# willi-menapace/PlayableEnvironments

Measured on AMD Instinct MI355X. Metric: Mrays/s, higher is better.
Workload: dtype f32; 1 GPU; tennis renderer, 256x256 frame per GPU (rank r renders the frame of seed 1234 + r), 4 objects, 64+128 hierarchical samples/ray (coarse+fine networks), eval - BASELINE.json configs[1]; rays_per_gpu=65536, frames_per_gpu=1, parallelism=frame shard x1

## Files before the change

### playableenvironments_amd/csrc/composite.hip

```cpp
#include "pr_common.h"
#include "composite_dev.h"

namespace pr {

struct CompositeSmem {
    float* tt;
    float* sg;
    float* dm;
    float* wo;
    float* wg;
    float* al;
    float* dv;
    int* sl;
    unsigned int* key;
};

constexpr int MAX_FCHUNK = 4;

__device__ __forceinline__ void transmittance_weights(float* al, int n, int lane) {
    float carry = 1.0f;
    for (int base = 0; base < n; base += 64) {
        const int j = base + lane;
        const float a = (j < n) ? al[j] : 0.f;
        float incl = (j < n) ? __fadd_rn(__fsub_rn(1.0f, a), 1e-10f) : 1.0f;
// ... 28 lines not shown
        const float a = (j < end) ? al[j] : 0.f;
        float incl = (j < end) ? __fadd_rn(__fsub_rn(1.0f, a), 1e-10f) : 1.0f;
#pragma unroll
        for (int d = 1; d < 64; d <<= 1) {
            const float o = __shfl_up(incl, d, 64);
            if (lane >= d) incl *= o;
        }
        float excl = __shfl_up(incl, 1, 64);
        if (lane == 0) excl = 1.0f;
        if (j < end) al[j] = a * (carry * excl);
        carry *= __shfl(incl, 63, 64);
    }
    if (lane == 0) totals[wave] = carry;
    __syncthreads();
    float before = 1.0f;
    for (int w = 0; w < wave; ++w) before *= totals[w];
    if (wave > 0)
        for (int j = begin + lane; j < end; j += 64) al[j] *= before;
    __syncthreads();
}

template <int CW>
__device__ __forceinline__ float block_sum(float v, float* scratch, int wave, int lane) {
    v = wave_sum(v);
    if (CW == 1) return v;
    __syncthreads();
    if (lane == 0) scratch[wave] = v;
    __syncthreads();
    float total = 0.f;
    for (int w = 0; w < CW; ++w) total += scratch[w];
    return total;
}

template <int CW>
__device__ __forceinline__ void store_channel_sums(float (&acc)[MAX_FCHUNK], float* dst, int F, float* scratch, int wave, int lane) {
    if (CW > 1) {
#pragma unroll
        for (int c = 0; c < MAX_FCHUNK; ++c) {
            if (64 * c >= F) break;
            __syncthreads();
            scratch[wave * 64 + lane] = acc[c];
            __syncthreads();
            if (wave == 0)
                for (int w = 1; w < CW; ++w) acc[c] = __fadd_rn(acc[c], scratch[w * 64 + lane]);
        }
    }
    if (wave == 0) {
#pragma unroll
        for (int c = 0; c < MAX_FCHUNK; ++c) {
            const int ch = lane + 64 * c;
            if (ch < F) dst[ch] = acc[c];
        }
    }
}

template <int CW>
__global__ __launch_bounds__(64 * CW) void k_composite(CompositeParams p) {
    extern __shared__ __attribute__((aligned(16))) char raw_smem[];
    constexpr int CT = 64 * CW;
    const int S = p.sort_size;
    CompositeSmem sm;
    const int A = (p.total_positions + 63) & ~63;
    sm.key = reinterpret_cast<unsigned int*>(raw_smem);
    sm.tt = reinterpret_cast<float*>(sm.key + S);
    sm.sg = sm.tt + A;
    sm.dm = sm.sg + A;
    sm.wo = sm.dm + A;
    sm.wg = sm.sg;
    sm.al = sm.wo + A;
    const bool use_div = p.any_divergence != 0;
    sm.dv = use_div ? sm.al + A : nullptr;
    sm.sl = reinterpret_cast<int*>(sm.al + (use_div ? 2 * A : A));
    float* scratch = reinterpret_cast<float*>(sm.sl + A);
    unsigned long long* wide = p.fix_overlaps ? reinterpret_cast<unsigned long long*>(scratch + 4 * 64) : nullptr;

    const int tid = threadIdx.x, lane = tid & 63;
    const int wave = (CW == 1) ? 0 : __builtin_amdgcn_readfirstlane(tid >> 6);
    const long g = blockIdx.x;
    const float* d = p.ray_directions + (size_t)g * 3;
    const float norm = sqrtf(__fadd_rn(__fadd_rn(__fmul_rn(d[0], d[0]), __fmul_rn(d[1], d[1])), __fmul_rn(d[2], d[2])));
    const int PT = p.total_positions;

    {
        int off = 0;
        for (int k = 0; k < p.objects; ++k) {
// ... 116 lines not shown
        sm.al[j] = alpha_of(raw, __fmul_rn(dt, norm));
        if (use_div) gdiv += sm.al[j] * sm.dv[e];
    }
    __syncthreads();
    transmittance_weights_block<CW>(sm.al, PT, scratch, wave, lane);
    if (CW == 1) __syncthreads();
    {
        float depth = 0.f, opacity = 0.f, dmag = 0.f;
        for (int j = tid; j < PT; j += CT) {
            const int e = (int)sm.key[j];
            const float w = sm.al[j];
            sm.wg[e] = w;
            if (p.global.weights) p.global.weights[gbase + j] = w;
            depth += w * sm.tt[e];
            opacity += w;
            dmag += w * sm.dm[e];
        }
        depth = block_sum<CW>(depth, scratch, wave, lane);
        opacity = block_sum<CW>(opacity, scratch, wave, lane);
        dmag = block_sum<CW>(dmag, scratch, wave, lane);
        if (use_div) gdiv = block_sum<CW>(gdiv, scratch, wave, lane);
        if (tid == 0) {
            if (p.global.depth) p.global.depth[g] = depth;
            if (p.global.opacity) p.global.opacity[g] = opacity;
            if (p.global.disparity) p.global.disparity[g] = disparity_of(depth, opacity);
            if (p.global.integrated_displacements_magnitude)
                p.global.integrated_displacements_magnitude[g] = dmag / (float)PT;
            if (p.global.integrated_divergence) p.global.integrated_divergence[g] = gdiv / (float)PT;
        }
    }
    __syncthreads();

    const int F = p.F;
    const bool defer = p.pooled != nullptr;
    int* lrow = reinterpret_cast<int*>(sm.key);
    float* lw1 = sm.tt;
    float accg[MAX_FCHUNK];
#pragma unroll
    for (int c = 0; c < MAX_FCHUNK; ++c) accg[c] = 0.f;
    int off = 0;
    for (int k = 0; k < p.objects; ++k) {
        const CompositeObject& o = p.obj[k];
        const int P = o.positions;
        const int part = (((P + CW - 1) / CW) + 63) & ~63;
        const int begin = wave * part;
        const int end = (begin + part < P) ? begin + part : P;
        __syncthreads();
        int count = 0;
        float bare1 = 0.f, bare2 = 0.f;
        for (int base = begin; base < end; base += 64) {
            const int i = base + lane;
            bool take = false;
            int row = -1;
            float w1 = 0.f, w2 = 0.f;
            if (i < end) {
                row = sm.sl[off + i];
                w1 = sm.wo[off + i];
                w2 = sm.wg[off + i];
                take = row >= 0 && (w1 != 0.f || w2 != 0.f);
                if (p.sigmoid && row < 0) {
                    bare1 += w1;
                    bare2 += w2;
                }
            }
            const unsigned long long m = __ballot(take);
            if (take) {
                const int pos = off + begin + count + __popcll(m & ((1ull << lane) - 1ull));
                lrow[pos] = row;
                lw1[pos] = w1;
                sm.al[pos] = w2;
            }
            count += __popcll(m);
        }
        const int* rows_w = lrow + off + begin;
        const float* w1_w = lw1 + off + begin;
        const float* w2_w = sm.al + off + begin;
        float acco[MAX_FCHUNK];
#pragma unroll
        for (int c = 0; c < MAX_FCHUNK; ++c) acco[c] = 0.f;
        int i = 0;
        for (; i + ROWS_IN_FLIGHT <= count; i += ROWS_IN_FLIGHT) {
            float v[ROWS_IN_FLIGHT][MAX_FCHUNK];
#pragma unroll
            for (int u = 0; u < ROWS_IN_FLIGHT; ++u) {
                const float* f = o.feat + (size_t)rows_w[i + u] * F;
#pragma unroll
                for (int c = 0; c < MAX_FCHUNK; ++c) {
                    const int ch = lane + 64 * c;
                    v[u][c] = (ch < F) ? f[ch] : 0.f;
                    if (p.sigmoid) v[u][c] = sigmoid_of(v[u][c]);
                }
            }
#pragma unroll
            for (int u = 0; u < ROWS_IN_FLIGHT; ++u) {
                const float w1 = w1_w[i + u], w2 = w2_w[i + u];
#pragma unroll
                for (int c = 0; c < MAX_FCHUNK; ++c) {
                    acco[c] = __fadd_rn(acco[c], __fmul_rn(w1, v[u][c]));
                    accg[c] = __fadd_rn(accg[c], __fmul_rn(w2, v[u][c]));
                }
            }
        }
        for (; i < count; ++i) {
            const float* f = o.feat + (size_t)rows_w[i] * F;
            const float w1 = w1_w[i], w2 = w2_w[i];
#pragma unroll
            for (int c = 0; c < MAX_FCHUNK; ++c) {
                const int ch = lane + 64 * c;
                float v = (ch < F) ? f[ch] : 0.f;
                if (p.sigmoid) v = sigmoid_of(v);
                acco[c] = __fadd_rn(acco[c], __fmul_rn(w1, v));
                accg[c] = __fadd_rn(accg[c], __fmul_rn(w2, v));
            }
        }
        if (p.sigmoid) {
            bare1 = wave_sum(bare1);
            bare2 = wave_sum(bare2);
#pragma unroll
            for (int c = 0; c < MAX_FCHUNK; ++c) {
                acco[c] = __fadd_rn(acco[c], 0.5f * bare1);
                accg[c] = __fadd_rn(accg[c], 0.5f * bare2);
            }
        }
        if (o.out.integrated_features)
            store_channel_sums<CW>(acco, defer ? p.pooled + ((size_t)(2 * k) * gridDim.x + g) * F : o.out.integrated_features + (size_t)g * F, F,
                                   scratch, wave, lane);
        if (defer) {
            if (p.global.integrated_features || p.decoder.groups > 0)
                store_channel_sums<CW>(accg, p.pooled + ((size_t)(2 * k + 1) * gridDim.x + g) * F, F, scratch, wave, lane);
#pragma unroll
            for (int c = 0; c < MAX_FCHUNK; ++c) accg[c] = 0.f;
        }
        off += P;
    }
    if (defer) return;
    if (p.global.integrated_features) store_channel_sums<CW>(accg, p.global.integrated_features + (size_t)g * F, F, scratch, wave, lane);
    if (p.decoder.groups > 0) {
        if (CW > 1 && !p.global.integrated_features) {
#pragma unroll
            for (int c = 0; c < MAX_FCHUNK; ++c) {
                if (64 * c >= F) break;
                __syncthreads();
                scratch[wave * 64 + lane] = accg[c];
                __syncthreads();
                if (wave == 0)
                    for (int w = 1; w < CW; ++w) accg[c] = __fadd_rn(accg[c], scratch[w * 64 + lane]);
            }
        }
        if (wave == 0) {
            const int frame = (int)(g / p.rays);
            int r = (int)(g - (long)frame * p.rays);
            int grp = 0;
            while (grp < p.decoder.groups - 1 && r >= p.decoder.rays[grp]) r -= p.decoder.rays[grp++];
            const int c0 = p.decoder.channel_begin[grp], c1 = p.decoder.channel_end[grp];
            const size_t cells = (size_t)p.decoder.rays[grp];
            float* map = p.decoder.map[grp] + (size_t)frame * (c1 - c0) * cells + r;
#pragma unroll
            for (int c = 0; c < MAX_FCHUNK; ++c) {
                const int ch = lane + 64 * c;
                if (ch >= c0 && ch < c1 && ch < F) map[(size_t)(ch - c0) * cells] = accg[c];
            }
        }
    }
}

int launch_composite(const CompositeParams& p, hipStream_t s) {
    PR_REQUIRE(p.F <= 64 * MAX_FCHUNK, "output_features %d exceeds %d", p.F, 64 * MAX_FCHUNK);
    PR_REQUIRE(p.sort_size >= p.total_positions && (p.sort_size & (p.sort_size - 1)) == 0, "bad sort size");
    for (int k = 0; k < p.objects; ++k)
        PR_REQUIRE(p.obj[k].positions <= 64 * 32, "positions per ray %d too large for the overlap mask", p.obj[k].positions);
    const size_t lds = (size_t)p.sort_size * 4 + (size_t)((p.total_positions + 63) & ~63) * (p.any_divergence ? 7 : 6) * 4 +
                       sizeof(float) * 4 * 64 + (p.fix_overlaps ? (size_t)p.sort_size * 8 : 0);
    PR_REQUIRE(lds <= 156 * 1024, "too many samples per ray for the compositing kernel (%d)", p.total_positions);
    if (p.decoder.groups > 0) {
        PR_REQUIRE(p.decoder.groups <= PR_MAX_DECODER_GROUPS, "decoder layout: %d groups (max %d)", p.decoder.groups, PR_MAX_DECODER_GROUPS);
        long sum = 0;
        for (int i = 0; i < p.decoder.groups; ++i) {
            PR_REQUIRE(p.decoder.rays[i] > 0 && p.decoder.width[i] > 0 && p.decoder.rays[i] % p.decoder.width[i] == 0,
                       "decoder layout: group %d has %d rays in rows of %d", i, p.decoder.rays[i], p.decoder.width[i]);
            PR_REQUIRE(p.decoder.channel_begin[i] >= 0 && p.decoder.channel_begin[i] < p.decoder.channel_end[i] && p.decoder.channel_end[i] <= (p.pooled ? p.out_features : p.F),
                       "decoder layout: group %d channel range [%d, %d) outside 0..%d", i, p.decoder.channel_begin[i], p.decoder.channel_end[i], p.pooled ? p.out_features : p.F);
            PR_REQUIRE(p.decoder.map[i] != nullptr, "decoder layout: group %d has no map", i);
            sum += p.decoder.rays[i];
        }
        PR_REQUIRE(sum == p.rays, "decoder layout: the groups hold %ld rays, the call has %d", sum, p.rays);
    }
    const long total = (long)p.frames * p.rays;
    ProfileScope scope(1, s);
    if (p.total_positions >= 256) {
        PR_TRY(prepare_kernel(reinterpret_cast<const void*>(&k_composite<4>), 156 * 1024, nullptr));
        hipLaunchKernelGGL(k_composite<4>, dim3((unsigned)total), dim3(256), lds, s, p);
    } else {
// ... 109 lines not shown
```

### playableenvironments_amd/csrc/geometry.hip

```cpp
#include "pr_common.h"

namespace pr {

__global__ void k_camera_rays(int frames, int rays, int per_frame, float half_h, float half_w, const float* __restrict__ c2w,
                              const float* __restrict__ focals, const int32_t* __restrict__ rows,
                              const int32_t* __restrict__ cols, float* __restrict__ origins,
                              float* __restrict__ dirs, float* __restrict__ normals) {
    const long g = (long)blockIdx.x * blockDim.x + threadIdx.x;
    const long total = (long)frames * rays;
    if (g >= total) return;
    const int n = (int)(g / rays);
    const int r = (int)(g - (long)n * rays);
    const float* m = c2w + (size_t)n * 12;
    const float f = focals[n];
    const long pix = per_frame ? g : (long)r;
    const float dx = __fdiv_rn(__fsub_rn((float)cols[pix], half_w), f);
    const float dy = -__fdiv_rn(__fsub_rn((float)rows[pix], half_h), f);
    const float dz = -1.0f;
#pragma unroll
    for (int i = 0; i < 3; ++i) {
        const float v = __fadd_rn(__fadd_rn(__fmul_rn(dx, m[i * 4 + 0]), __fmul_rn(dy, m[i * 4 + 1])),
                                  __fmul_rn(dz, m[i * 4 + 2]));
        dirs[g * 3 + i] = v;
    }
// ... 283 lines not shown
    PR_LAUNCH_CHECK();
    hipLaunchKernelGGL(k_fill_group, dim3(blocks, count), dim3(256), 0, s, fg);
    PR_LAUNCH_CHECK();
    return PR_OK;
}

int launch_fill(const FillParams& p, hipStream_t s) {
    const long total = (long)p.frames * p.rays;
    const int blocks = (int)((total + 255) / 256);
    hipLaunchKernelGGL(k_fill, dim3(blocks), dim3(256), 0, s, p);
    PR_LAUNCH_CHECK();
    return PR_OK;
}

__device__ __forceinline__ void bitonic_sort_f32(float* key, int n , int lane) {
    for (int k = 2; k <= n; k <<= 1) {
        for (int j = k >> 1; j > 0; j >>= 1) {
            for (int i = lane; i < n; i += 64) {
                const int x = i ^ j;
                if (x > i) {
                    const float a = key[i], b = key[x];
                    const bool up = ((i & k) == 0);
                    if ((a > b) == up) {
                        key[i] = b;
                        key[x] = a;
                    }
                }
            }
            __syncthreads();
        }
    }
}

__global__ __launch_bounds__(64) void k_resample(ResampleParams p, int sort_size) {
    extern __shared__ float sm[];
    if (p.skip && *p.skip) return;
    const int Pc = p.pc, Pf = p.pf;
    float* tc = sm;
    float* al = tc + Pc;
    float* mids = al + Pc;
    float* cdf = mids + Pc;
    float* key = cdf + Pc;
    const int lane = threadIdx.x;
    const long g = blockIdx.x;
    const int n = (int)(g / p.rays);
    const float* m = p.w2o + ((size_t)n * p.objects + p.object_index) * 12;
    const ObjRay ray = object_ray(m, p.ray_origins + (size_t)n * 3, p.ray_directions + (size_t)g * 3);
    const bool valid = p.in_scene[(size_t)n * p.objects + p.object_index] != 0;
    const float norm = sqrtf(__fadd_rn(__fadd_rn(__fmul_rn(ray.d[0], ray.d[0]), __fmul_rn(ray.d[1], ray.d[1])),
                                       __fmul_rn(ray.d[2], ray.d[2])));
    const size_t cbase = (size_t)g * Pc;
    for (int i = lane; i < Pc; i += 64) tc[i] = p.t_coarse[cbase + i];
    __syncthreads();
    for (int i = lane; i < Pc; i += 64) {
        float raw = valid ? p.sigma_coarse[cbase + i] : p.empty_alpha;
        if (noise_present(p.alpha_noise)) raw = __fadd_rn(raw, noise_normal(p.alpha_noise, g, Pc, i));
        const float dt = (i < Pc - 1) ? __fsub_rn(tc[i + 1], tc[i]) : 1e10f;
        const float dist = __fmul_rn(dt, norm);
        const float relu = raw > 0.f ? raw : 0.f;
        al[i] = __fsub_rn(1.0f, expf(__fmul_rn(-relu, dist)));
        if (i < Pc - 1) mids[i] = __fdiv_rn(__fadd_rn(tc[i + 1], tc[i]), 2.0f);
    }
    __syncthreads();
    if (lane == 0) {
        float trans = 1.0f;
        for (int i = 0; i < Pc; ++i) {
            const float a = al[i];
            al[i] = __fmul_rn(a, trans);
            trans = __fmul_rn(trans, __fadd_rn(__fsub_rn(1.0f, a), 1e-10f));
        }
        const int nb = Pc - 2;
        float sum = 0.f;
        for (int j = 0; j < nb; ++j) sum = __fadd_rn(sum, __fadd_rn(al[j + 1], 1e-5f));
        float c = 0.f;
        cdf[0] = 0.f;
        for (int j = 0; j < nb; ++j) {
            c = __fadd_rn(c, __fdiv_rn(__fadd_rn(al[j + 1], 1e-5f), sum));
            cdf[j + 1] = c;
        }
    }
    __syncthreads();
    const int ncdf = Pc - 1;
    for (int i = lane; i < sort_size; i += 64) key[i] = (i < Pc) ? tc[i] : __builtin_inff();
    for (int f = lane; f < Pf; f += 64) {
        const float u = noise_present(p.u_random) ? noise_uniform(p.u_random, g, Pf, f) : p.u_fixed[f];
        int lo_i = 0, hi_i = ncdf;
        while (lo_i < hi_i) {
            const int mid = (lo_i + hi_i) >> 1;
            if (cdf[mid] > u) hi_i = mid; else lo_i = mid + 1;
        }
        const int below = lo_i - 1 < 0 ? 0 : lo_i - 1;
        const int above = lo_i > ncdf - 1 ? ncdf - 1 : lo_i;
        float den = __fsub_rn(cdf[above], cdf[below]);
        if (den < 1e-5f) den = 1.0f;
        const float frac = __fdiv_rn(__fsub_rn(u, cdf[below]), den);
        key[Pc + f] = __fadd_rn(mids[below], __fmul_rn(frac, __fsub_rn(mids[above], mids[below])));
    }
    __syncthreads();
    const int Pm = Pc + Pf;
    float* merged = key + sort_size;
    bool sorted = true;
    for (int i = lane; i + 1 < Pc; i += 64) sorted = sorted && (key[i] <= key[i + 1]);
    for (int f = lane; f + 1 < Pf; f += 64) sorted = sorted && (key[Pc + f] <= key[Pc + f + 1]);
    if (__ballot(sorted) == ~0ull) {
        for (int i = lane; i < Pc; i += 64) {
            const float t = key[i];
            int lo = 0, hi = Pf;
            while (lo < hi) {
                const int mid = (lo + hi) >> 1;
                if (key[Pc + mid] < t) lo = mid + 1; else hi = mid;
            }
            merged[i + lo] = t;
        }
        for (int f = lane; f < Pf; f += 64) {
            const float t = key[Pc + f];
            int lo = 0, hi = Pc;
            while (lo < hi) {
                const int mid = (lo + hi) >> 1;
                if (key[mid] <= t) lo = mid + 1; else hi = mid;
            }
            merged[f + lo] = t;
        }
        __syncthreads();
    } else {
        bitonic_sort_f32(key, sort_size, lane);
        merged = key;
    }
    const size_t fbase = (size_t)g * Pm;
    int count = 0;
    for (int i = lane; i < Pm; i += 64) {
        const float t = merged[i];
        p.t_fine[fbase + i] = t;
        p.sigma_fine[fbase + i] = p.empty_alpha;
        if (p.dispmag_fine) p.dispmag_fine[fbase + i] = 0.f;
        const float x = __fadd_rn(ray.o[0], __fmul_rn(ray.d[0], t));
        const float y = __fadd_rn(ray.o[1], __fmul_rn(ray.d[1], t));
        const float z = __fadd_rn(ray.o[2], __fmul_rn(ray.d[2], t));
        if (sample_kept(x, y, z, p.lo, p.hi, p.occ, n)) ++count;
    }
#pragma unroll
    for (int d = 32; d > 0; d >>= 1) count += __shfl_down(count, d, 64);
    if (lane == 0 && count) atomicAdd(&p.block_sums[g >> 8], count);
}

__global__ __launch_bounds__(256) void k_expected_positions(int frames, int rays, int objects, int object_index, int P,
                                                            const float* ray_origins, const float* ray_directions,
                                                            const float* w2o, const float* t, const float* weights,
                                                            const float* delta, float* expected) {
    const long g = (long)blockIdx.x * 256 + threadIdx.x;
    if (g >= (long)frames * rays) return;
    const int n = (int)(g / rays);
    const ObjRay ray = object_ray(w2o + ((size_t)n * objects + object_index) * 12, ray_origins + (size_t)n * 3,
                                  ray_directions + (size_t)g * 3);
    const size_t base = (size_t)g * P;
    float acc[3] = {0.f, 0.f, 0.f}, wsum = 0.f;
    for (int i = 0; i < P; ++i) {
        const float ti = t[base + i], w = weights[base + i];
        for (int a = 0; a < 3; ++a) {
            float x = __fadd_rn(ray.o[a], __fmul_rn(ray.d[a], ti));
            if (delta) x = __fadd_rn(x, delta[(base + i) * 3 + a]);
            acc[a] = __fadd_rn(acc[a], __fmul_rn(x, w));
        }
        wsum = __fadd_rn(wsum, w);
    }
    for (int a = 0; a < 3; ++a) expected[(size_t)g * 3 + a] = __fdiv_rn(acc[a], __fadd_rn(wsum, 1e-8f));
}

static int next_pow2(int v) {
    int r = 1;
    while (r < v) r <<= 1;
    return r;
}

int launch_resample(const ResampleParams& p, hipStream_t s) {
    PR_REQUIRE(p.pc >= 3, "hierarchical sampling needs at least 3 coarse positions (got %d)", p.pc);
    const long total = (long)p.frames * p.rays;
    const int nblocks256 = (int)((total + 255) / 256);
    PR_TRY(launch_zero_fill(p.block_sums, sizeof(int32_t) * nblocks256, s));
    int sort_size = next_pow2(p.pc + p.pf);
    if (sort_size < 64) sort_size = 64;
    const size_t lds = sizeof(float) * (4 * (size_t)p.pc + 2 * (size_t)sort_size);
    PR_REQUIRE(lds <= 64 * 1024, "resample: too many positions per ray (%d + %d)", p.pc, p.pf);
    hipLaunchKernelGGL(k_resample, dim3((unsigned)total), dim3(64), lds, s, p, sort_size);
    PR_LAUNCH_CHECK();
    return PR_OK;
}

}

extern "C" int pr_expected_positions(int32_t frames, int32_t rays, int32_t objects, int32_t object_index, int32_t positions,
                                     const float* ray_origins, const float* ray_directions, const float* w2o, const float* t,
                                     const float* weights, const float* delta, float* expected, void* stream) {
    PR_REQUIRE(frames > 0 && rays > 0 && positions > 0 && objects > 0 && object_index >= 0 && object_index < objects,
               "pr_expected_positions: bad sizes");
    PR_REQUIRE(ray_origins && ray_directions && w2o && t && weights && expected, "pr_expected_positions: NULL pointer");
    const long total = (long)frames * rays;
    hipLaunchKernelGGL(pr::k_expected_positions, dim3((unsigned)((total + 255) / 256)), dim3(256), 0, (hipStream_t)stream, frames,
                       rays, objects, object_index, positions, ray_origins, ray_directions, w2o, t, weights, delta, expected);
    PR_LAUNCH_CHECK();
    return PR_OK;
}

namespace pr {
struct PatchPixelsParams {
    int frames, objects, height, width, patch, nstrides;
    int strides[4];
    const float* boxes;
    const float* weights;
    const float* u;
    int32_t* rows; int32_t* cols;
    int rays;
};

__global__ __launch_bounds__(256) void k_patch_pixels(PatchPixelsParams p) {
    __shared__ int start[2];
    const int n = blockIdx.x;
// ... 457 lines not shown
```

### playableenvironments_amd/csrc/pr_common.h

```cpp
#pragma once

#include <hip/hip_runtime.h>
#include <stdint.h>
#include <stdio.h>
#include <string.h>

#include "playrender.h"

namespace pr {

void set_error(const char* fmt, ...);

#define PR_CHECK_HIP(expr)                                                              \
    do {                                                                                \
        hipError_t _e = (expr);                                                         \
        if (_e != hipSuccess) {                                                         \
            pr::set_error("%s failed: %s (%s:%d)", #expr, hipGetErrorString(_e), __FILE__, __LINE__); \
            return PR_ERR_HIP;                                                          \
        }                                                                               \
    } while (0)

#define PR_REQUIRE(cond, ...)                                                           \
    do {                                                                                \
        if (!(cond)) {                                                                  \
// ... 266 lines not shown
    float* rec_pos;
    int32_t* rec_flat;
    int32_t* slot;
    OccGrid occ;
    const int32_t* skip;
};
int launch_fill(const FillParams& p, hipStream_t s);
int launch_placement_group(const PlaceParams* pp, const FillParams* fp, int32_t* const* totals, int count, hipStream_t s);

int launch_scan(const int32_t* sums, int32_t* offsets, int32_t* total, int n, hipStream_t s);

struct ResampleParams {
    int frames, rays, objects, object_index;
    int pc, pf;
    const float* ray_origins;
    const float* ray_directions;
    const float* w2o;
    const uint8_t* in_scene;
    float lo[3], hi[3];
    float empty_alpha;
    const float* t_coarse;
    const float* sigma_coarse;
    NoiseRef alpha_noise;
    const float* u_fixed;
    NoiseRef u_random;
    float* t_fine;
    float* sigma_fine;
    float* dispmag_fine;
    int32_t* block_sums;
    OccGrid occ;
    const int32_t* skip;
};
int launch_resample(const ResampleParams& p, hipStream_t s);

struct FoldParams {
    int frames, objects, object_index;
    const float* style;
    int S;
    pr_linear_t affine1; const float* bn1_mean; const float* bn1_var;
    pr_linear_t affine4; const float* bn4_mean; const float* bn4_var;
    float eps;
    int W, Wpad, W2, W2pad;
    float* table;
    int row_floats;
};
int launch_adain_fold(const FoldParams& p, hipStream_t s);
int launch_adain_fold_group(const FoldParams* jobs, int count, hipStream_t s);

int launch_mlp(const MlpParams& p, int max_rows, bool naive, const pr_object_model_t* raw, hipStream_t s);
int launch_mlp_group(const MlpParams* host_jobs, const int* max_rows, int count, hipStream_t s);
int launch_mlp_split(const MlpParams& p, int max_rows, int terms, hipStream_t s);
int launch_mlp_split_group(const MlpParams* host_jobs, const int* max_rows, int count, int terms, hipStream_t s);
int launch_mlp_sigma(const MlpParams& p, int max_rows, hipStream_t s);
int launch_mlp_split_sigma(const MlpParams& p, int max_rows, int terms, hipStream_t s);

struct BnFinalizeParams {
    const double* stats;
    const int32_t* count;
    int width, width_pad;
    float momentum;
    float* running_mean;
    float* running_var;
    long long* num_batches_tracked;
    float* batch_mean;
    float* batch_var;
    int frozen;
// ... 376 lines not shown
```

### playableenvironments_amd/csrc/render.hip

```cpp
#include "pr_common.h"

#include <stdarg.h>

#include <atomic>
#include <mutex>
#include <vector>

namespace pr {

struct ProfileRecord { int category; hipEvent_t start, stop; };
static std::atomic<bool> g_profile_on{false};
static std::vector<ProfileRecord> g_profile;
static std::mutex g_profile_mutex;

int prepare_kernel(const void* kernel, int lds_bytes, int* cu_count) {
    struct Entry { const void* kernel; int device; int cus; };
    static std::vector<Entry> done;
    static std::mutex guard;
    int dev = 0;
    PR_CHECK_HIP(hipGetDevice(&dev));
    std::lock_guard<std::mutex> lock(guard);
    for (const Entry& e : done)
        if (e.kernel == kernel && e.device == dev) {
            if (cu_count) *cu_count = e.cus;
// ... 255 lines not shown
    }
}

struct SampleArrays { float* t; float* sigma; int32_t* slot; float* dispmag; float* feat; };
static SampleArrays sample_arrays(const Plan& plan, char* ws, const RetainCtx* rc, int t, int k, bool has_bender) {
    SampleArrays a;
    if (rc && ((rc->mask >> k) & 1u)) {
        const RetainObjectPlan& o = rc->plan.obj[k];
        a.t = reinterpret_cast<float*>(rc->base + o.t[t]);
        a.sigma = reinterpret_cast<float*>(rc->base + o.sigma[t]);
        a.slot = reinterpret_cast<int32_t*>(rc->base + o.slot[t]);
        a.dispmag = has_bender ? reinterpret_cast<float*>(rc->base + o.dispmag[t]) : nullptr;
        a.feat = reinterpret_cast<float*>(rc->base + o.feat[t]);
        return a;
    }
    const TypePlan& tp = plan.type[t];
    a.t = reinterpret_cast<float*>(ws + tp.t[k]);
    a.sigma = reinterpret_cast<float*>(ws + tp.sigma[k]);
    a.slot = reinterpret_cast<int32_t*>(ws + tp.slot[k]);
    a.dispmag = has_bender ? reinterpret_cast<float*>(ws + tp.dispmag[k]) : nullptr;
    a.feat = reinterpret_cast<float*>(ws + tp.feat[k]);
    return a;
}

static int render(const pr_call_t& c, const pr_object_t* objs, const pr_occupancy_t* occupancy, const RetainCtx* rc,
                  const pr_outputs_t* outs[2], char* ws, const Plan& plan, hipStream_t s) {
    const int ntypes = c.use_fine ? 2 : 1;
    const int K = c.objects;
    if (rc) PR_TRY(launch_retain_probe(c, objs, *rc, s));
    int32_t* block_sums_all = reinterpret_cast<int32_t*>(ws + plan.block_sums);
    int32_t* block_offsets_all = reinterpret_cast<int32_t*>(ws + plan.block_offsets);
    const bool place_grouped = c.objects > 1 && ((c.flags & PR_FLAG_SAVE_FOR_BACKWARD) || group_active(c));
    static thread_local PlaceParams place_jobs[PR_MAX_OBJECTS];
    static thread_local FillParams fill_jobs[PR_MAX_OBJECTS];
    int32_t* total_ptrs[PR_MAX_OBJECTS];
    float* rec_pos = reinterpret_cast<float*>(ws + plan.rec_pos);
    int32_t* rec_flat = reinterpret_cast<int32_t*>(ws + plan.rec_flat);
    const bool naive = (c.flags & PR_FLAG_NAIVE_MLP) != 0;
    const bool gate = gate_active(c);
    const bool defer = defer_active(c, objs);
    const bool grouped = group_active(c);
    MlpParams jobs[PR_MAX_OBJECTS];
    int job_rows[PR_MAX_OBJECTS];
    FoldParams fold_jobs[PR_MAX_OBJECTS];
    const bool train_grouped = group_train_active(c);
    struct TrainJob {
        MlpParams mp; FoldParams fo; ModelDims d; const pr_object_model_t* m; const SavedPlan* sv;
        double* stats; int32_t* stat_count; float* batch; float* h1; float* h2; float* rec_pos; int32_t* rec_flat;
        int k, P, max_tiles; bool frozen, save;
    };
    static thread_local TrainJob train_jobs[PR_MAX_OBJECTS];

    for (int t = 0; t < ntypes; ++t) {
        const TypePlan& tp = plan.type[t];
        int32_t* totals = reinterpret_cast<int32_t*>(ws + tp.totals);
        int32_t* head_counts = reinterpret_cast<int32_t*>(ws + tp.head_counts);
        PR_TRY(launch_zero_fill(ws + tp.zero_begin, tp.zero_bytes, s));
        const pr_noise_t& noise = t ? c.noise_fine : c.noise_coarse;
        int total_positions = 0;
        auto finish_object = [&](TrainJob& J, int stage, bool launch) -> int {
            MlpParams& mp = J.mp; FoldParams& fo = J.fo; const ModelDims& d = J.d; const pr_object_model_t& m = *J.m;
            const SavedPlan& sv = *J.sv;
            double* stats = J.stats; int32_t* stat_count = J.stat_count; float* batch = J.batch; float* h1 = J.h1; float* h2 = J.h2;
            float* rec_pos = J.rec_pos; int32_t* rec_flat = J.rec_flat;
            const int k = J.k, P = J.P, max_tiles = J.max_tiles;
            const bool frozen = J.frozen, save = J.save;
// ... 23 lines not shown
                mp.phase = 3; mp.h_in = h2; mp.h_in_width = d.W2pad; mp.h_out = nullptr;
                if (launch) PR_TRY(launch_mlp(mp, max_tiles, false, &m, s));
                return PR_OK;
            }
            if (outs[t] && outs[t]->normalised_samples)
                PR_CHECK_HIP(hipMemcpyAsync(outs[t]->normalised_samples + k, stat_count, sizeof(int32_t),
                                            hipMemcpyDeviceToDevice, s));
            if (save && m.has_bender) {
                const size_t cap_rows = (size_t)c.frames * c.rays * P;
                float* div = reinterpret_cast<float*>(ws + sv.div);
                NoiseRef probes = make_noise(noise.divergence[k], c, NOISE_DIVERGENCE, t, k);
                if (!(c.flags & PR_FLAG_TRAIN_BN)) probes.generate = 0;
                if (probes.ptr || probes.generate) {
                    DivergenceParams dp;
                    memset(&dp, 0, sizeof(dp));
                    dp.total = totals + k; dp.max_rows = (int)cap_rows;
                    dp.rec_flat = rec_flat; dp.row_flags = mp.row_flags; dp.rec_pos = rec_pos;
                    dp.noise = probes; dp.positions = P;
                    dp.bin = mp.save_bin; dp.bin_pad = d.bin_pad; dp.benc = d.benc; dp.b_octaves = m.bender_octaves;
                    dp.bacts = mp.save_bact; dp.bact_stride = mp.save_bact_stride; dp.BW = d.BW; dp.BWpad = d.BWpad;
                    dp.b_count = m.bender_count; dp.b_skip = m.bender_skip; dp.bin_real = d.bin;
                    dp.layers = m.bender; dp.out_head = m.bender_out; dp.braw = mp.save_braw;
                    bbox_split(m, dp.lo, dp.hi, nullptr);
                    dp.canonical = (c.flags & PR_FLAG_CANONICAL_POSE) ? 1 : 0;
                    dp.t0 = reinterpret_cast<float*>(ws + plan.div_t0);
                    dp.ta = reinterpret_cast<float*>(ws + plan.div_ta);
                    dp.tb = reinterpret_cast<float*>(ws + plan.div_tb);
                    dp.div = div;
                    PR_TRY(launch_divergence(dp, s));
                }
            }
            return PR_OK;
        };
        for (int pass = (place_grouped && t == 0) ? 0 : 1; pass < 2; ++pass) {
        if (pass == 1 && place_grouped && t == 0) PR_TRY(launch_placement_group(place_jobs, fill_jobs, total_ptrs, K, s));
        for (int k = 0; k < K; ++k) {
            const pr_object_model_t& m = t ? objs[k].fine : objs[k].coarse;
            const float* packed = static_cast<const float*>(t ? objs[k].packed_fine : objs[k].packed_coarse);
            ModelDims d;
            PackedLayout l;
            PR_TRY(compute_dims(m, &d));
            PR_TRY(compute_layout(m, d, &l));
            const int P = m.positions;
            if (pass == 1) total_positions += P;
            int32_t* block_sums = block_sums_all + (size_t)k * plan.nblocks256;
            int32_t* block_offsets = block_offsets_all + (size_t)k * plan.nblocks256;
            const bool placed = place_grouped && t == 0;
            const SampleArrays arr = sample_arrays(plan, ws, rc, t, k, m.has_bender != 0);
            float* t_arr = arr.t;
            float* sigma = arr.sigma;
            int32_t* slot = arr.slot;
            float* dispmag = arr.dispmag;
            float* feat = arr.feat;
            const int32_t* skip = (rc && ((rc->mask >> k) & 1u)) ? &rc->hdr->reuse[k] : nullptr;
            float* adain = reinterpret_cast<float*>(ws + tp.adain[k]);
            const bool save = (c.flags & PR_FLAG_SAVE_FOR_BACKWARD) != 0;
            const SavedPlan& sv = tp.saved[k];
            OccGrid occ;
            PR_TRY(make_occ_grid(occupancy ? (t ? &occupancy->fine[k] : &occupancy->coarse[k]) : nullptr, m, k, t ? "fine" : "coarse", &occ));
            if (save) {
                rec_pos = reinterpret_cast<float*>(ws + sv.rec_pos);
                rec_flat = reinterpret_cast<int32_t*>(ws + sv.rec_flat);
            } else if (grouped) {
                rec_pos = reinterpret_cast<float*>(ws + plan.rec_pos_k[k]);
                rec_flat = reinterpret_cast<int32_t*>(ws + plan.rec_flat_k[k]);
            }

            if (t == 0) {
                PlaceParams pp;
                memset(&pp, 0, sizeof(pp));
                pp.frames = c.frames; pp.rays = c.rays; pp.positions = P; pp.objects = K; pp.object_index = k;
                pp.ray_origins = c.ray_origins; pp.ray_directions = c.ray_directions; pp.w2o = c.w2o;
                pp.in_scene = c.object_in_scene;
                bbox_split(m, pp.lo, pp.hi, nullptr);
                pp.z_near_min = m.z_near_min; pp.z_far_max = m.z_far_max; pp.empty_alpha = m.empty_space_alpha;
                pp.linspace = c.linspace_coarse[k];
                pp.jitter = perturb_noise(c.noise_coarse.jitter[k], c, NOISE_JITTER, 0, k);
                pp.t = t_arr; pp.sigma = sigma; pp.dispmag = dispmag; pp.block_sums = block_sums;
                pp.occ = occ;
                pp.skip = skip;
                if (pass == 0) place_jobs[k] = pp;
                else if (!placed) PR_TRY(launch_place_coarse(pp, s));
            } else {
                ResampleParams rp;
                memset(&rp, 0, sizeof(rp));
                rp.frames = c.frames; rp.rays = c.rays; rp.objects = K; rp.object_index = k;
                rp.pc = objs[k].coarse.positions; rp.pf = c.positions_fine[k];
                rp.ray_origins = c.ray_origins; rp.ray_directions = c.ray_directions; rp.w2o = c.w2o;
                rp.in_scene = c.object_in_scene;
                bbox_split(m, rp.lo, rp.hi, nullptr);
                rp.empty_alpha = m.empty_space_alpha;
                const SampleArrays coarse_arr = sample_arrays(plan, ws, rc, 0, k, objs[k].coarse.has_bender != 0);
                rp.t_coarse = coarse_arr.t;
                rp.sigma_coarse = coarse_arr.sigma;
                rp.alpha_noise = perturb_noise(c.noise_coarse.alpha[k], c, NOISE_ALPHA, 0, k);
                rp.u_fixed = c.linspace_fine[k];
                rp.u_random = perturb_noise(c.noise_coarse.pdf[k], c, NOISE_PDF, 0, k);
                rp.t_fine = t_arr; rp.sigma_fine = sigma; rp.dispmag_fine = dispmag; rp.block_sums = block_sums;
                rp.occ = occ;
                rp.skip = skip;
                PR_TRY(launch_resample(rp, s));
            }
            if (pass == 1 && !placed) PR_TRY(launch_scan(block_sums, block_offsets, totals + k, plan.nblocks256, s));

            FillParams fp;
            memset(&fp, 0, sizeof(fp));
            fp.frames = c.frames; fp.rays = c.rays; fp.positions = P; fp.objects = K; fp.object_index = k;
            fp.ray_origins = c.ray_origins; fp.ray_directions = c.ray_directions; fp.w2o = c.w2o;
            fp.in_scene = c.object_in_scene;
            bbox_split(m, fp.lo, fp.hi, nullptr);
            fp.t = t_arr; fp.block_offsets = block_offsets; fp.rec_pos = rec_pos; fp.rec_flat = rec_flat; fp.slot = slot;
            fp.occ = occ;
            fp.skip = skip;
            if (pass == 0) {
                fill_jobs[k] = fp;
                total_ptrs[k] = totals + k;
                continue;
            }
            if (!placed) PR_TRY(launch_fill(fp, s));

            FoldParams fo;
            memset(&fo, 0, sizeof(fo));
            fo.frames = c.frames; fo.objects = K; fo.object_index = k;
            fo.style = c.style; fo.S = m.style_features;
            fo.affine1 = m.affine1; fo.bn1_mean = m.bn1_mean; fo.bn1_var = m.bn1_var;
            fo.affine4 = m.affine4; fo.bn4_mean = m.bn4_mean; fo.bn4_var = m.bn4_var;
            fo.eps = m.bn_eps;
            fo.W = d.W; fo.Wpad = d.Wpad; fo.W2 = d.W2; fo.W2pad = d.W2pad;
            fo.table = adain; fo.row_floats = adain_row_floats(d);

            MlpParams mp;
            memset(&mp, 0, sizeof(mp));
            const bool split3 = train_grouped && (c.flags & PR_FLAG_SPLIT_BACKWARD) && (c.flags & PR_FLAG_SAVE_FOR_BACKWARD);
            PR_TRY(build_mlp_layers(m, d, l, packed, &mp, split3));
// ... 388 lines not shown
```

Before: 0.3297 Mrays/s.

## Vectorize composite feature gathers, batch rays per resample block, group resample launches

When the feature width is a multiple of four, the composite kernel now gathers features with one 16-byte load per lane and keeps seven rows in flight in a software pipeline, replacing per-channel strided loads. The resample kernel now handles up to four rays per block, sized by an LDS budget, and a grouped launch runs resample, scan and fill for all objects in a few launches instead of one set per object. The aim is to cut global-load instruction count and kernel-launch overhead and to raise occupancy of the small resample blocks. In exchange the composite channel-to-lane mapping changes and resample blocks run more serial per-ray work.

```diff
diff --git a/playableenvironments_amd/csrc/composite.hip b/playableenvironments_amd/csrc/composite.hip
--- a/playableenvironments_amd/csrc/composite.hip
+++ b/playableenvironments_amd/csrc/composite.hip
@@ -84,12 +84,14 @@
     return total;
 }
 
+__device__ __forceinline__ int channel_of(int lane, int c, bool quad) { return quad ? 4 * lane + c : lane + 64 * c; }
+
 template <int CW>
-__device__ __forceinline__ void store_channel_sums(float (&acc)[MAX_FCHUNK], float* dst, int F, float* scratch, int wave, int lane) {
+__device__ __forceinline__ void add_channel_sums(float (&acc)[MAX_FCHUNK], int F, bool quad, float* scratch, int wave, int lane) {
     if (CW > 1) {
 #pragma unroll
         for (int c = 0; c < MAX_FCHUNK; ++c) {
-            if (64 * c >= F) break;
+            if (!quad && 64 * c >= F) break;
             __syncthreads();
             scratch[wave * 64 + lane] = acc[c];
             __syncthreads();
@@ -97,12 +99,65 @@
                 for (int w = 1; w < CW; ++w) acc[c] = __fadd_rn(acc[c], scratch[w * 64 + lane]);
         }
     }
+}
+
+template <int CW>
+__device__ __forceinline__ void store_channel_sums(float (&acc)[MAX_FCHUNK], float* dst, int F, bool quad, float* scratch, int wave, int lane) {
+    add_channel_sums<CW>(acc, F, quad, scratch, wave, lane);
     if (wave == 0) {
 #pragma unroll
         for (int c = 0; c < MAX_FCHUNK; ++c) {
-            const int ch = lane + 64 * c;
+            const int ch = channel_of(lane, c, quad);
             if (ch < F) dst[ch] = acc[c];
         }
+    }
+}
+
+constexpr int QUAD_ROWS_IN_FLIGHT = 7;
+template <bool SIGMOID>
+__device__ __forceinline__ void add_rows_quad(const float* feat, int F, const int* rows, const float* w1s, const float* w2s, int count,
+                                              int lane, float (&acco)[MAX_FCHUNK], float (&accg)[MAX_FCHUNK]) {
+    constexpr int R = QUAD_ROWS_IN_FLIGHT;
+    auto request = [&](int i) {
+        const int row = __builtin_amdgcn_readfirstlane(rows[i]);
+        const char* base = reinterpret_cast<const char*>(feat + (size_t)row * F);
+        return *reinterpret_cast<const PR_GLOBAL_AS f32x4_t*>(as_global(base) + (unsigned)lane * 16u);
+    };
+    auto add = [&](f32x4_t v, int i) {
+        const float w1 = w1s[i], w2 = w2s[i];
+#pragma unroll
+        for (int c = 0; c < 4; ++c) {
+            const float x = SIGMOID ? sigmoid_of(v[c]) : v[c];
+            acco[c] = __fadd_rn(acco[c], __fmul_rn(w1, x));
+            accg[c] = __fadd_rn(accg[c], __fmul_rn(w2, x));
+        }
+        asm volatile("" : "+v"(acco[0]), "+v"(acco[1]), "+v"(acco[2]), "+v"(acco[3]), "+v"(accg[0]), "+v"(accg[1]), "+v"(accg[2]), "+v"(accg[3]));
+    };
+    int i = 0;
+    if (count >= R) {
+        f32x4_t v[R];
+#pragma unroll
+        for (int u = 0; u < R; ++u) v[u] = request(u);
+        for (; i + 2 * R <= count; i += R) {
+#pragma unroll
+            for (int u = 0; u < R; ++u) {
+                add(v[u], i + u);
+                v[u] = request(i + R + u);
+                __builtin_amdgcn_sched_barrier(0);
+            }
+        }
+#pragma unroll
+        for (int u = 0; u < R; ++u) add(v[u], i + u);
+        i += R;
+    }
+    if (i < count) {
+        f32x4_t v[R - 1];
+#pragma unroll
+        for (int u = 0; u < R - 1; ++u)
+            if (i + u < count) v[u] = request(i + u);
+#pragma unroll
+        for (int u = 0; u < R - 1; ++u)
+            if (i + u < count) add(v[u], i + u);
     }
 }
 
@@ -285,6 +340,7 @@
     __syncthreads();
 
     const int F = p.F;
+    const bool quad = (F & 3) == 0;
     const bool defer = p.pooled != nullptr;
     int* lrow = reinterpret_cast<int*>(sm.key);
     float* lw1 = sm.tt;
@@ -331,39 +387,47 @@
         float acco[MAX_FCHUNK];
 #pragma unroll
         for (int c = 0; c < MAX_FCHUNK; ++c) acco[c] = 0.f;
-        int i = 0;
-        for (; i + ROWS_IN_FLIGHT <= count; i += ROWS_IN_FLIGHT) {
-            float v[ROWS_IN_FLIGHT][MAX_FCHUNK];
-#pragma unroll
-            for (int u = 0; u < ROWS_IN_FLIGHT; ++u) {
-                const float* f = o.feat + (size_t)rows_w[i + u] * F;
-#pragma unroll
+        if (quad) {
+            if (4 * lane < F) {
+                if (p.sigmoid) add_rows_quad<true>(o.feat, F, rows_w, w1_w, w2_w, count, lane, acco, accg);
+                else add_rows_quad<false>(o.feat, F, rows_w, w1_w, w2_w, count, lane, acco, accg);
+            }
+        } else {
+            int i = 0;
+            for (; i + ROWS_IN_FLIGHT <= count; i += ROWS_IN_FLIGHT) {
+                float v[ROWS_IN_FLIGHT][MAX_FCHUNK];
+    #pragma unroll
+                for (int u = 0; u < ROWS_IN_FLIGHT; ++u) {
+                    const float* f = o.feat + (size_t)rows_w[i + u] * F;
+    #pragma unroll
+                    for (int c = 0; c < MAX_FCHUNK; ++c) {
+                        const int ch = lane + 64 * c;
+                        v[u][c] = (ch < F) ? f[ch] : 0.f;
+                        if (p.sigmoid) v[u][c] = sigmoid_of(v[u][c]);
+                    }
+                }
+    #pragma unroll
+                for (int u = 0; u < ROWS_IN_FLIGHT; ++u) {
+                    const float w1 = w1_w[i + u], w2 = w2_w[i + u];
+    #pragma unroll
+                    for (int c = 0; c < MAX_FCHUNK; ++c) {
+                        acco[c] = __fadd_rn(acco[c], __fmul_rn(w1, v[u][c]));
+                        accg[c] = __fadd_rn(accg[c], __fmul_rn(w2, v[u][c]));
+                    }
+                    asm volatile("" : "+v"(acco[0]), "+v"(acco[1]), "+v"(acco[2]), "+v"(acco[3]), "+v"(accg[0]), "+v"(accg[1]), "+v"(accg[2]), "+v"(accg[3]));
+                }
+            }
+            for (; i < count; ++i) {
+                const float* f = o.feat + (size_t)rows_w[i] * F;
+                const float w1 = w1_w[i], w2 = w2_w[i];
+    #pragma unroll
                 for (int c = 0; c < MAX_FCHUNK; ++c) {
                     const int ch = lane + 64 * c;
-                    v[u][c] = (ch < F) ? f[ch] : 0.f;
-                    if (p.sigmoid) v[u][c] = sigmoid_of(v[u][c]);
-                }
-            }
-#pragma unroll
-            for (int u = 0; u < ROWS_IN_FLIGHT; ++u) {
-                const float w1 = w1_w[i + u], w2 = w2_w[i + u];
-#pragma unroll
-                for (int c = 0; c < MAX_FCHUNK; ++c) {
-                    acco[c] = __fadd_rn(acco[c], __fmul_rn(w1, v[u][c]));
-                    accg[c] = __fadd_rn(accg[c], __fmul_rn(w2, v[u][c]));
-                }
-            }
-        }
-        for (; i < count; ++i) {
-            const float* f = o.feat + (size_t)rows_w[i] * F;
-            const float w1 = w1_w[i], w2 = w2_w[i];
-#pragma unroll
-            for (int c = 0; c < MAX_FCHUNK; ++c) {
-                const int ch = lane + 64 * c;
-                float v = (ch < F) ? f[ch] : 0.f;
-                if (p.sigmoid) v = sigmoid_of(v);
-                acco[c] = __fadd_rn(acco[c], __fmul_rn(w1, v));
-                accg[c] = __fadd_rn(accg[c], __fmul_rn(w2, v));
+                    float v = (ch < F) ? f[ch] : 0.f;
+                    if (p.sigmoid) v = sigmoid_of(v);
+                    acco[c] = __fadd_rn(acco[c], __fmul_rn(w1, v));
+                    accg[c] = __fadd_rn(accg[c], __fmul_rn(w2, v));
+                }
             }
         }
         if (p.sigmoid) {
@@ -377,29 +441,19 @@
         }
         if (o.out.integrated_features)
             store_channel_sums<CW>(acco, defer ? p.pooled + ((size_t)(2 * k) * gridDim.x + g) * F : o.out.integrated_features + (size_t)g * F, F,
-                                   scratch, wave, lane);
+                                   quad, scratch, wave, lane);
         if (defer) {
             if (p.global.integrated_features || p.decoder.groups > 0)
-                store_channel_sums<CW>(accg, p.pooled + ((size_t)(2 * k + 1) * gridDim.x + g) * F, F, scratch, wave, lane);
+                store_channel_sums<CW>(accg, p.pooled + ((size_t)(2 * k + 1) * gridDim.x + g) * F, F, quad, scratch, wave, lane);
 #pragma unroll
             for (int c = 0; c < MAX_FCHUNK; ++c) accg[c] = 0.f;
         }
         off += P;
     }
     if (defer) return;
-    if (p.global.integrated_features) store_channel_sums<CW>(accg, p.global.integrated_features + (size_t)g * F, F, scratch, wave, lane);
+    if (p.global.integrated_features) store_channel_sums<CW>(accg, p.global.integrated_features + (size_t)g * F, F, quad, scratch, wave, lane);
     if (p.decoder.groups > 0) {
-        if (CW > 1 && !p.global.integrated_features) {
-#pragma unroll
-            for (int c = 0; c < MAX_FCHUNK; ++c) {
-                if (64 * c >= F) break;
-                __syncthreads();
-                scratch[wave * 64 + lane] = accg[c];
-                __syncthreads();
-                if (wave == 0)
-                    for (int w = 1; w < CW; ++w) accg[c] = __fadd_rn(accg[c], scratch[w * 64 + lane]);
-            }
-        }
+        if (!p.global.integrated_features) add_channel_sums<CW>(accg, F, quad, scratch, wave, lane);
         if (wave == 0) {
             const int frame = (int)(g / p.rays);
             int r = (int)(g - (long)frame * p.rays);
@@ -410,7 +464,7 @@
             float* map = p.decoder.map[grp] + (size_t)frame * (c1 - c0) * cells + r;
 #pragma unroll
             for (int c = 0; c < MAX_FCHUNK; ++c) {
-                const int ch = lane + 64 * c;
+                const int ch = channel_of(lane, c, quad);
                 if (ch >= c0 && ch < c1 && ch < F) map[(size_t)(ch - c0) * cells] = accg[c];
             }
         }
diff --git a/playableenvironments_amd/csrc/geometry.hip b/playableenvironments_amd/csrc/geometry.hip
--- a/playableenvironments_amd/csrc/geometry.hip
+++ b/playableenvironments_amd/csrc/geometry.hip
@@ -339,37 +339,54 @@
     }
 }
 
-__global__ __launch_bounds__(64) void k_resample(ResampleParams p, int sort_size) {
+constexpr int RESAMPLE_RAYS = 4;
+__device__ __forceinline__ void resample_body(const ResampleParams& p, int sort_size, int rpg) {
     extern __shared__ float sm[];
-    if (p.skip && *p.skip) return;
+    if (p.skip && *as_global(p.skip)) return;
     const int Pc = p.pc, Pf = p.pf;
-    float* tc = sm;
-    float* al = tc + Pc;
-    float* mids = al + Pc;
-    float* cdf = mids + Pc;
-    float* key = cdf + Pc;
+    const int per_ray = 4 * Pc + 2 * sort_size;
     const int lane = threadIdx.x;
-    const long g = blockIdx.x;
-    const int n = (int)(g / p.rays);
-    const float* m = p.w2o + ((size_t)n * p.objects + p.object_index) * 12;
-    const ObjRay ray = object_ray(m, p.ray_origins + (size_t)n * 3, p.ray_directions + (size_t)g * 3);
-    const bool valid = p.in_scene[(size_t)n * p.objects + p.object_index] != 0;
-    const float norm = sqrtf(__fadd_rn(__fadd_rn(__fmul_rn(ray.d[0], ray.d[0]), __fmul_rn(ray.d[1], ray.d[1])),
-                                       __fmul_rn(ray.d[2], ray.d[2])));
-    const size_t cbase = (size_t)g * Pc;
-    for (int i = lane; i < Pc; i += 64) tc[i] = p.t_coarse[cbase + i];
+    const long total = (long)p.frames * p.rays;
+    const long g0 = (long)blockIdx.x * rpg;
+    if (g0 >= total) return;
+    const int here = (int)((total - g0 < rpg) ? total - g0 : rpg);
+    auto ray_of = [&](long g, int* n, bool* valid) {
+        *n = (int)(g / p.rays);
+        const float* m = p.w2o + ((size_t)*n * p.objects + p.object_index) * 12;
+        *valid = p.in_scene[(size_t)*n * p.objects + p.object_index] != 0;
+        return object_ray(m, p.ray_origins + (size_t)*n * 3, p.ray_directions + (size_t)g * 3);
+    };
+    for (int r = 0; r < here; ++r) {
+        float* tc = sm + (size_t)r * per_ray;
+        const size_t cbase = (size_t)(g0 + r) * Pc;
+        for (int i = lane; i < Pc; i += 64) tc[i] = as_global(p.t_coarse)[cbase + i];
+    }
     __syncthreads();
-    for (int i = lane; i < Pc; i += 64) {
-        float raw = valid ? p.sigma_coarse[cbase + i] : p.empty_alpha;
-        if (noise_present(p.alpha_noise)) raw = __fadd_rn(raw, noise_normal(p.alpha_noise, g, Pc, i));
-        const float dt = (i < Pc - 1) ? __fsub_rn(tc[i + 1], tc[i]) : 1e10f;
-        const float dist = __fmul_rn(dt, norm);
-        const float relu = raw > 0.f ? raw : 0.f;
-        al[i] = __fsub_rn(1.0f, expf(__fmul_rn(-relu, dist)));
-        if (i < Pc - 1) mids[i] = __fdiv_rn(__fadd_rn(tc[i + 1], tc[i]), 2.0f);
+    for (int r = 0; r < here; ++r) {
+        float* tc = sm + (size_t)r * per_ray;
+        float* al = tc + Pc;
+        float* mids = al + Pc;
+        const long g = g0 + r;
+        int n;
+        bool valid;
+        const ObjRay ray = ray_of(g, &n, &valid);
+        const float norm = sqrtf(__fadd_rn(__fadd_rn(__fmul_rn(ray.d[0], ray.d[0]), __fmul_rn(ray.d[1], ray.d[1])),
+                                           __fmul_rn(ray.d[2], ray.d[2])));
+        const size_t cbase = (size_t)g * Pc;
+        for (int i = lane; i < Pc; i += 64) {
+            float raw = valid ? as_global(p.sigma_coarse)[cbase + i] : p.empty_alpha;
+            if (noise_present(p.alpha_noise)) raw = __fadd_rn(raw, noise_normal(p.alpha_noise, g, Pc, i));
+            const float dt = (i < Pc - 1) ? __fsub_rn(tc[i + 1], tc[i]) : 1e10f;
+            const float dist = __fmul_rn(dt, norm);
+            const float relu = raw > 0.f ? raw : 0.f;
+            al[i] = __fsub_rn(1.0f, expf(__fmul_rn(-relu, dist)));
+            if (i < Pc - 1) mids[i] = __fdiv_rn(__fadd_rn(tc[i + 1], tc[i]), 2.0f);
+        }
     }
     __syncthreads();
-    if (lane == 0) {
+    if (lane < here) {
+        float* al = sm + (size_t)lane * per_ray + Pc;
+        float* cdf = al + 2 * Pc;
         float trans = 1.0f;
         for (int i = 0; i < Pc; ++i) {
             const float a = al[i];
@@ -388,66 +405,86 @@
     }
     __syncthreads();
     const int ncdf = Pc - 1;
-    for (int i = lane; i < sort_size; i += 64) key[i] = (i < Pc) ? tc[i] : __builtin_inff();
-    for (int f = lane; f < Pf; f += 64) {
-        const float u = noise_present(p.u_random) ? noise_uniform(p.u_random, g, Pf, f) : p.u_fixed[f];
-        int lo_i = 0, hi_i = ncdf;
-        while (lo_i < hi_i) {
-            const int mid = (lo_i + hi_i) >> 1;
-            if (cdf[mid] > u) hi_i = mid; else lo_i = mid + 1;
-        }
-        const int below = lo_i - 1 < 0 ? 0 : lo_i - 1;
-        const int above = lo_i > ncdf - 1 ? ncdf - 1 : lo_i;
-        float den = __fsub_rn(cdf[above], cdf[below]);
-        if (den < 1e-5f) den = 1.0f;
-        const float frac = __fdiv_rn(__fsub_rn(u, cdf[below]), den);
-        key[Pc + f] = __fadd_rn(mids[below], __fmul_rn(frac, __fsub_rn(mids[above], mids[below])));
+    for (int r = 0; r < here; ++r) {
+        float* tc = sm + (size_t)r * per_ray;
+        float* mids = tc + 2 * Pc;
+        float* cdf = mids + Pc;
+        float* key = cdf + Pc;
+        const long g = g0 + r;
+        for (int i = lane; i < sort_size; i += 64) key[i] = (i < Pc) ? tc[i] : __builtin_inff();
+        for (int f = lane; f < Pf; f += 64) {
+            const float u = noise_present(p.u_random) ? noise_uniform(p.u_random, g, Pf, f) : as_global(p.u_fixed)[f];
+            int lo_i = 0, hi_i = ncdf;
+            while (lo_i < hi_i) {
+                const int mid = (lo_i + hi_i) >> 1;
+                if (cdf[mid] > u) hi_i = mid; else lo_i = mid + 1;
+            }
+            const int below = lo_i - 1 < 0 ? 0 : lo_i - 1;
+            const int above = lo_i > ncdf - 1 ? ncdf - 1 : lo_i;
+            float den = __fsub_rn(cdf[above], cdf[below]);
+            if (den < 1e-5f) den = 1.0f;
+            const float frac = __fdiv_rn(__fsub_rn(u, cdf[below]), den);
+            key[Pc + f] = __fadd_rn(mids[below], __fmul_rn(frac, __fsub_rn(mids[above], mids[below])));
+        }
     }
     __syncthreads();
     const int Pm = Pc + Pf;
-    float* merged = key + sort_size;
-    bool sorted = true;
-    for (int i = lane; i + 1 < Pc; i += 64) sorted = sorted && (key[i] <= key[i + 1]);
-    for (int f = lane; f + 1 < Pf; f += 64) sorted = sorted && (key[Pc + f] <= key[Pc + f + 1]);
-    if (__ballot(sorted) == ~0ull) {
-        for (int i = lane; i < Pc; i += 64) {
-            const float t = key[i];
-            int lo = 0, hi = Pf;
-            while (lo < hi) {
-                const int mid = (lo + hi) >> 1;
-                if (key[Pc + mid] < t) lo = mid + 1; else hi = mid;
+    int count = 0;
+    for (int r = 0; r < here; ++r) {
+        float* key = sm + (size_t)r * per_ray + 4 * Pc;
+        const long g = g0 + r;
+        float* merged = key + sort_size;
+        bool sorted = true;
+        for (int i = lane; i + 1 < Pc; i += 64) sorted = sorted && (key[i] <= key[i + 1]);
+        for (int f = lane; f + 1 < Pf; f += 64) sorted = sorted && (key[Pc + f] <= key[Pc + f + 1]);
+        if (__ballot(sorted) == ~0ull) {
+            for (int i = lane; i < Pc; i += 64) {
+                const float t = key[i];
+                int lo = 0, hi = Pf;
+                while (lo < hi) {
+                    const int mid = (lo + hi) >> 1;
+                    if (key[Pc + mid] < t) lo = mid + 1; else hi = mid;
+                }
+                merged[i + lo] = t;
             }
-            merged[i + lo] = t;
-        }
-        for (int f = lane; f < Pf; f += 64) {
-            const float t = key[Pc + f];
-            int lo = 0, hi = Pc;
-            while (lo < hi) {
-                const int mid = (lo + hi) >> 1;
-                if (key[mid] <= t) lo = mid + 1; else hi = mid;
+            for (int f = lane; f < Pf; f += 64) {
+                const float t = key[Pc + f];
+                int lo = 0, hi = Pc;
+                while (lo < hi) {
+                    const int mid = (lo + hi) >> 1;
+                    if (key[mid] <= t) lo = mid + 1; else hi = mid;
+                }
+                merged[f + lo] = t;
             }
-            merged[f + lo] = t;
-        }
-        __syncthreads();
-    } else {
-        bitonic_sort_f32(key, sort_size, lane);
-        merged = key;
-    }
-    const size_t fbase = (size_t)g * Pm;
-    int count = 0;
-    for (int i = lane; i < Pm; i += 64) {
-        const float t = merged[i];
-        p.t_fine[fbase + i] = t;
-        p.sigma_fine[fbase + i] = p.empty_alpha;
-        if (p.dispmag_fine) p.dispmag_fine[fbase + i] = 0.f;
-        const float x = __fadd_rn(ray.o[0], __fmul_rn(ray.d[0], t));
-        const float y = __fadd_rn(ray.o[1], __fmul_rn(ray.d[1], t));
-        const float z = __fadd_rn(ray.o[2], __fmul_rn(ray.d[2], t));
-        if (sample_kept(x, y, z, p.lo, p.hi, p.occ, n)) ++count;
+            __syncthreads();
+        } else {
+            bitonic_sort_f32(key, sort_size, lane);
+            merged = key;
+        }
+        int n;
+        bool valid;
+        const ObjRay ray = ray_of(g, &n, &valid);
+        const size_t fbase = (size_t)g * Pm;
+        for (int i = lane; i < Pm; i += 64) {
+            const float t = merged[i];
+            p.t_fine[fbase + i] = t;
+            p.sigma_fine[fbase + i] = p.empty_alpha;
+            if (p.dispmag_fine) p.dispmag_fine[fbase + i] = 0.f;
+            const float x = __fadd_rn(ray.o[0], __fmul_rn(ray.d[0], t));
+            const float y = __fadd_rn(ray.o[1], __fmul_rn(ray.d[1], t));
+            const float z = __fadd_rn(ray.o[2], __fmul_rn(ray.d[2], t));
+            if (sample_kept(x, y, z, p.lo, p.hi, p.occ, n)) ++count;
+        }
     }
 #pragma unroll
     for (int d = 32; d > 0; d >>= 1) count += __shfl_down(count, d, 64);
-    if (lane == 0 && count) atomicAdd(&p.block_sums[g >> 8], count);
+    if (lane == 0 && count) atomicAdd(&p.block_sums[g0 >> 8], count);
+}
+
+__global__ __launch_bounds__(64) void k_resample(ResampleParams p, int sort_size, int rpg) { resample_body(p, sort_size, rpg); }
+struct ResampleGroup { ResampleParams p[PR_MAX_OBJECTS]; int sort_size[PR_MAX_OBJECTS]; int rpg[PR_MAX_OBJECTS]; };
+__global__ __launch_bounds__(64) void k_resample_group(ResampleGroup g) {
+    resample_body(g.p[blockIdx.y], g.sort_size[blockIdx.y], g.rpg[blockIdx.y]);
 }
 
 __global__ __launch_bounds__(256) void k_expected_positions(int frames, int rays, int objects, int object_index, int P,
@@ -479,16 +516,60 @@
     return r;
 }
 
+static int resample_shape(const ResampleParams& p, int* sort_size, int* rpg, size_t* lds) {
+    PR_REQUIRE(p.pc >= 3, "hierarchical sampling needs at least 3 coarse positions (got %d)", p.pc);
+    *sort_size = next_pow2(p.pc + p.pf);
+    if (*sort_size < 64) *sort_size = 64;
+    const size_t per_ray = sizeof(float) * (4 * (size_t)p.pc + 2 * (size_t)*sort_size);
+    PR_REQUIRE(per_ray <= 64 * 1024, "resample: too many positions per ray (%d + %d)", p.pc, p.pf);
+    *rpg = RESAMPLE_RAYS;
+    while (*rpg > 1 && per_ray * *rpg > 16 * 1024) *rpg >>= 1;
+    *lds = per_ray * *rpg;
+    return PR_OK;
+}
+
 int launch_resample(const ResampleParams& p, hipStream_t s) {
-    PR_REQUIRE(p.pc >= 3, "hierarchical sampling needs at least 3 coarse positions (got %d)", p.pc);
+    int sort_size, rpg;
+    size_t lds;
+    PR_TRY(resample_shape(p, &sort_size, &rpg, &lds));
     const long total = (long)p.frames * p.rays;
     const int nblocks256 = (int)((total + 255) / 256);
     PR_TRY(launch_zero_fill(p.block_sums, sizeof(int32_t) * nblocks256, s));
-    int sort_size = next_pow2(p.pc + p.pf);
-    if (sort_size < 64) sort_size = 64;
-    const size_t lds = sizeof(float) * (4 * (size_t)p.pc + 2 * (size_t)sort_size);
-    PR_REQUIRE(lds <= 64 * 1024, "resample: too many positions per ray (%d + %d)", p.pc, p.pf);
-    hipLaunchKernelGGL(k_resample, dim3((unsigned)total), dim3(64), lds, s, p, sort_size);
+    hipLaunchKernelGGL(k_resample, dim3((unsigned)((total + rpg - 1) / rpg)), dim3(64), lds, s, p, sort_size, rpg);
+    PR_LAUNCH_CHECK();
+    return PR_OK;
+}
+
+int launch_resample_group(const ResampleParams* rp, const FillParams* fp, int32_t* const* totals, int32_t* sums, int count, hipStream_t s) {
+    if (count <= 0) return PR_OK;
+    PR_REQUIRE(count <= PR_MAX_OBJECTS, "resample group: %d objects", count);
+    static thread_local ResampleGroup rg;
+    static thread_local FillGroup fg;
+    ScanGroup sg;
+    const long total = (long)rp[0].frames * rp[0].rays;
+    const int blocks = (int)((total + 255) / 256);
+    size_t lds = 0;
+    long groups = 0;
+    for (int k = 0; k < count; ++k) {
+        size_t need;
+        PR_TRY(resample_shape(rp[k], &rg.sort_size[k], &rg.rpg[k], &need));
+        if (need > lds) lds = need;
+        const long mine = (total + rg.rpg[k] - 1) / rg.rpg[k];
+        if (mine > groups) groups = mine;
+        PR_REQUIRE(rp[k].block_sums == sums + (size_t)k * blocks, "resample group: object %d's block sums are not in the group's array", k);
+        rg.p[k] = rp[k];
+        fg.p[k] = fp[k];
+        sg.sums[k] = rp[k].block_sums;
+        sg.offsets[k] = const_cast<int32_t*>(fp[k].block_offsets);
+        sg.total[k] = totals[k];
+    }
+    sg.n = blocks;
+    PR_TRY(launch_zero_fill(sums, sizeof(int32_t) * (size_t)count * blocks, s));
+    hipLaunchKernelGGL(k_resample_group, dim3((unsigned)groups, count), dim3(64), lds, s, rg);
+    PR_LAUNCH_CHECK();
+    hipLaunchKernelGGL(k_scan_blocks_group, dim3(count), dim3(256), 0, s, sg);
+    PR_LAUNCH_CHECK();
+    hipLaunchKernelGGL(k_fill_group, dim3(blocks, count), dim3(256), 0, s, fg);
     PR_LAUNCH_CHECK();
     return PR_OK;
 }
diff --git a/playableenvironments_amd/csrc/pr_common.h b/playableenvironments_amd/csrc/pr_common.h
--- a/playableenvironments_amd/csrc/pr_common.h
+++ b/playableenvironments_amd/csrc/pr_common.h
@@ -322,6 +322,7 @@
     const int32_t* skip;
 };
 int launch_resample(const ResampleParams& p, hipStream_t s);
+int launch_resample_group(const ResampleParams* rp, const FillParams* fp, int32_t* const* totals, int32_t* sums, int count, hipStream_t s);
 
 struct FoldParams {
     int frames, objects, object_index;
diff --git a/playableenvironments_amd/csrc/render.hip b/playableenvironments_amd/csrc/render.hip
--- a/playableenvironments_amd/csrc/render.hip
+++ b/playableenvironments_amd/csrc/render.hip
@@ -311,6 +311,7 @@
     int32_t* block_offsets_all = reinterpret_cast<int32_t*>(ws + plan.block_offsets);
     const bool place_grouped = c.objects > 1 && ((c.flags & PR_FLAG_SAVE_FOR_BACKWARD) || group_active(c));
     static thread_local PlaceParams place_jobs[PR_MAX_OBJECTS];
+    static thread_local ResampleParams resample_jobs[PR_MAX_OBJECTS];
     static thread_local FillParams fill_jobs[PR_MAX_OBJECTS];
     int32_t* total_ptrs[PR_MAX_OBJECTS];
     float* rec_pos = reinterpret_cast<float*>(ws + plan.rec_pos);
@@ -400,8 +401,11 @@
             }
             return PR_OK;
         };
-        for (int pass = (place_grouped && t == 0) ? 0 : 1; pass < 2; ++pass) {
-        if (pass == 1 && place_grouped && t == 0) PR_TRY(launch_placement_group(place_jobs, fill_jobs, total_ptrs, K, s));
+        for (int pass = place_grouped ? 0 : 1; pass < 2; ++pass) {
+        if (pass == 1 && place_grouped) {
+            if (t == 0) PR_TRY(launch_placement_group(place_jobs, fill_jobs, total_ptrs, K, s));
+            else PR_TRY(launch_resample_group(resample_jobs, fill_jobs, total_ptrs, block_sums_all, K, s));
+        }
         for (int k = 0; k < K; ++k) {
             const pr_object_model_t& m = t ? objs[k].fine : objs[k].coarse;
             const float* packed = static_cast<const float*>(t ? objs[k].packed_fine : objs[k].packed_coarse);
@@ -413,7 +417,7 @@
             if (pass == 1) total_positions += P;
             int32_t* block_sums = block_sums_all + (size_t)k * plan.nblocks256;
             int32_t* block_offsets = block_offsets_all + (size_t)k * plan.nblocks256;
-            const bool placed = place_grouped && t == 0;
+            const bool placed = place_grouped;
             const SampleArrays arr = sample_arrays(plan, ws, rc, t, k, m.has_bender != 0);
             float* t_arr = arr.t;
             float* sigma = arr.sigma;
@@ -467,7 +471,8 @@
                 rp.t_fine = t_arr; rp.sigma_fine = sigma; rp.dispmag_fine = dispmag; rp.block_sums = block_sums;
                 rp.occ = occ;
                 rp.skip = skip;
-                PR_TRY(launch_resample(rp, s));
+                if (pass == 0) resample_jobs[k] = rp;
+                else if (!placed) PR_TRY(launch_resample(rp, s));
             }
             if (pass == 1 && !placed) PR_TRY(launch_scan(block_sums, block_offsets, totals + k, plan.nblocks256, s));
 
```

Result: no change. 0.3315 Mrays/s (median of 6 runs) (+0.5%).
